# RandallBalestriero/noise-robust-vit

Hardware: AMD Instinct MI355X
Metric: images/sec (fwd+bwd+optimizer) ViT-B/16 224px bf16 (higher is better)
Workload: dtype bf16

## Files before the change

### noise_robust_vit_amd/csrc/nrv_attn.hip

```cpp
#include <type_traits>

#include "nrv_attn_common.hpp"

NRV_INTERNAL int nrv_attn_gen_supported(int B, int N, int H, int dh);
NRV_INTERNAL int nrv_attn_gen_fwd(const void* qkv, void* out, float* lse, int B, int N, int H, int dh, float scale, hipStream_t s);
NRV_INTERNAL int nrv_attn_gen_bwd(const void* qkv, const void* out, const void* dout, const float* lse, void* dqkv, float* delta_ws,
                     int B, int N, int H, int dh, float scale, hipStream_t s);
NRV_INTERNAL int nrv_attn_gen_probs(const void* qkv, const float* lse, float* probs, int B, int N, int H, int dh, float scale, hipStream_t s);

namespace {

using namespace nrv_attn;
struct AttnParams {
    const bf16_t* qkv;
    const bf16_t* out;
    const bf16_t* dout;
    bf16_t* o;
    bf16_t* dqkv;
    float* lse;
    float* delta;
    int B, N, H;
    float scale;
    long long q_rs, q_ws, q_hs, q_bs, o_rs, o_hs, o_bs;
};

void set_layout(AttnParams& p, int layout, int dh) {
    const long long T = (long long)p.B * p.N;
    if (layout & NRV_ATTN_QKV_BLOCKED) { p.q_rs = dh; p.q_ws = (long long)p.H * T * dh; p.q_hs = T * dh; p.q_bs = (long long)p.N * dh; }
    else { p.q_rs = 3ll * p.H * dh; p.q_ws = (long long)p.H * dh; p.q_hs = dh; p.q_bs = p.N * p.q_rs; }
    if (layout & NRV_ATTN_OUT_BLOCKED) { p.o_rs = dh; p.o_hs = T * dh; p.o_bs = (long long)p.N * dh; }
    else { p.o_rs = (long long)p.H * dh; p.o_hs = dh; p.o_bs = p.N * p.o_rs; }
}

template <int NT>
constexpr int atf_waves() { return NT <= 2 ? 1 : NT <= 4 ? 2 : 4; }

template <int NT>
__global__ __launch_bounds__(64 * atf_waves<NT>(), NT <= 13 ? 3 : 2) void attn_fwd_fat_kernel(const AttnParams p) {
    extern __shared__ __attribute__((aligned(16))) char smem[];
    constexpr int NP = NT * 16;
    constexpr int IMG = NP * 128;
    constexpr int NS = (NT + 1) / 2;
    constexpr int NJ = 2 * NP / 8;
    constexpr int ATF_WAVES = atf_waves<NT>();
    constexpr int JPW = NJ / ATF_WAVES;
    constexpr int MT = (NT == 13 || NT == 14) ? 1 : 2;
    const int tid = threadIdx.x, lane = tid & 63, wave = tid >> 6;
    const int N = p.N, H = p.H;
    const long long ldq = p.q_rs;
    const int b = blockIdx.x / H, h = blockIdx.x - b * H;
    const bf16_t* hb = p.qkv + (long long)b * p.q_bs + h * p.q_hs;
    const int g = lane >> 4, qc = lane & 15;
    const float sc = p.scale * LOG2E;
    const char* kimg = smem;
    const char* vimg = smem + IMG;

    const int npairs = (N + 31) >> 5;
    bf16x8_t qf[2][2];
    auto load_q = [&](int pair) {
#pragma unroll
        for (int t = 0; t < 2; ++t) {
            const int q = pair * 32 + t * 16 + qc;
            const int qr = q < N ? q : N - 1;
#pragma unroll
            for (int ks = 0; ks < 2; ++ks) qf[t][ks] = load_frag_global(hb + (long long)qr * ldq + ks * 32 + g * 8);
        }
    };
    if (wave < npairs) load_q(wave);
    {
        const __amdgpu_buffer_rsrc_t rk = make_rsrc(hb + p.q_ws, 0x7fffffffull), rv = make_rsrc(hb + 2 * p.q_ws, 0x7fffffffull);
        const int wave_u = __builtin_amdgcn_readfirstlane(wave);
#pragma unroll
        for (int i = 0; i < JPW; ++i) {
            const int j = wave_u * JPW + i;
            const bool isv = j >= NP / 8;
            const int r = 8 * (isv ? j - NP / 8 : j) + (lane >> 3);
            const int pos = lane & 7;
            const int c = isv ? ((((pos >> 1) ^ ((r >> 1) & 3)) << 1) | (pos & 1)) : (pos ^ ((r >> 1) & 7));
            const unsigned vo = (r < N) ? (unsigned)(r * ldq * 2 + c * 16) : NRV_OOB;
            if (isv) dma16_nt(rv, smem + j * 1024, vo);
            else dma16_nt(rk, smem + j * 1024, vo);
        }
    }
    __builtin_amdgcn_s_waitcnt(0x0F70);
    asm volatile("" ::: "memory");
    __syncthreads();

    const bf16x4_t zero4 = {0, 0, 0, 0};
    auto v_frag = [&](int kk, int dt) {
        const int q = (lane & 15) >> 2, pp = lane & 3;
        const int r0 = kk * 32 + 4 * g + q;
        const bf16x4_t lo = lds_read_tr16_b64(vimg + r0 * 128 + ((dt ^ ((r0 >> 1) & 3)) << 5) + pp * 8);
        if (2 * kk + 1 >= NT) return cat4(lo, zero4);
        return cat4(lo, lds_read_tr16_b64(vimg + (r0 + 16) * 128 + ((dt ^ (((r0 + 16) >> 1) & 3)) << 5) + pp * 8));
    };
    const int d_lane = (g & 1) ? 16 + 4 * (g - 1) : 4 * g;
    for (int pair = wave; pair < npairs; pair += ATF_WAVES) {
        f32x4_t st[2][NT];
        constexpr int KD = NT < 4 ? NT : 4;
        bf16x8_t kf[KD][2];
#pragma unroll
        for (int j = 0; j < KD - 1; ++j)
#pragma unroll
            for (int ks = 0; ks < 2; ++ks) kf[j][ks] = row_frag_img(kimg, j * 16, ks, lane);
#pragma unroll
        for (int kt = 0; kt < NT; ++kt) {
            if (kt + KD - 1 < NT) {
#pragma unroll
                for (int ks = 0; ks < 2; ++ks) kf[(kt + KD - 1) % KD][ks] = row_frag_img(kimg, (kt + KD - 1) * 16, ks, lane);
            }
#pragma unroll
            for (int t = 0; t < 2; ++t) {
                f32x4_t a = {0.f, 0.f, 0.f, 0.f};
#pragma unroll
                for (int ks = 0; ks < 2; ++ks) a = mfma16(kf[kt % KD][ks], qf[t][ks], a);
                st[t][kt] = a;
            }
        }
        __builtin_amdgcn_sched_barrier(0);
        const int q0 = pair * 32 + qc;
        if (pair + ATF_WAVES < npairs) load_q(pair + ATF_WAVES);
        bf16x8_t vf[2][4];
#pragma unroll
        for (int dt = 0; dt < 4; ++dt) vf[0][dt] = v_frag(0, dt);
        float m[2], l[2];
        bf16x8_t pf[2][NS];
#pragma unroll
        for (int t = 0; t < 2; ++t) {
            float mm = -INFINITY;
#pragma unroll
            for (int kt = 0; kt < NT; ++kt) {
#pragma unroll
                for (int e = 0; e < 4; ++e) {
                    if (kt >= NT - MT) mm = fmaxf(mm, (kt * 16 + 4 * g + e < N) ? st[t][kt][e] : -INFINITY);
                    else mm = fmaxf(mm, st[t][kt][e]);
                }
            }
            mm = fmaxf(mm, __shfl_xor(mm, 16, 64));
            mm = fmaxf(mm, __shfl_xor(mm, 32, 64));
            mm *= sc;
            float ll = 0.f;
#pragma unroll
            for (int kt = 0; kt < NT; ++kt) {
#pragma unroll
                for (int e = 0; e < 4; ++e) {
                    float pv = __builtin_amdgcn_exp2f(fmaf(st[t][kt][e], sc, -mm));
                    if (kt >= NT - MT) pv = (kt * 16 + 4 * g + e < N) ? pv : 0.f;
                    st[t][kt][e] = pv;
                    ll += pv;
                }
                if (kt & 1) pf[t][kt >> 1] = pack_frag(st[t][kt - 1], st[t][kt]);
                else if (kt == NT - 1) pf[t][kt >> 1] = pack_frag(st[t][kt], f32x4_t{0.f, 0.f, 0.f, 0.f});
            }
            ll += __shfl_xor(ll, 16, 64);
            ll += __shfl_xor(ll, 32, 64);
            m[t] = mm;
            l[t] = ll;
        }
        __builtin_amdgcn_sched_barrier(0);
        f32x4_t o[2][4];
#pragma unroll
        for (int t = 0; t < 2; ++t)
#pragma unroll
            for (int dt = 0; dt < 4; ++dt) o[t][dt] = f32x4_t{0.f, 0.f, 0.f, 0.f};
#pragma unroll
        for (int kk = 0; kk < NS; ++kk) {
            if (kk + 1 < NS) {
#pragma unroll
                for (int dt = 0; dt < 4; ++dt) vf[(kk + 1) & 1][dt] = v_frag(kk + 1, dt);
            }
#pragma unroll
            for (int dt = 0; dt < 4; ++dt)
#pragma unroll
                for (int t = 0; t < 2; ++t) o[t][dt] = mfma16(vf[kk & 1][dt], pf[t][kk], o[t][dt]);
        }
        __builtin_amdgcn_sched_barrier(0);
#pragma unroll
        for (int t = 0; t < 2; ++t) {
            const int q = q0 + t * 16;
            const float inv = 1.0f / l[t];
            u32x4_t ov[2];
#pragma unroll
            for (int pr = 0; pr < 2; ++pr) {
                const f32x4_t oa = o[t][2 * pr] * inv, ob = o[t][2 * pr + 1] * inv;
                const auto lo = __builtin_amdgcn_permlane16_swap(pack_bf16x2(oa[0], oa[1]), pack_bf16x2(ob[0], ob[1]), false, false);
                const auto hi = __builtin_amdgcn_permlane16_swap(pack_bf16x2(oa[2], oa[3]), pack_bf16x2(ob[2], ob[3]), false, false);
                ov[pr] = u32x4_t{lo[0], hi[0], lo[1], hi[1]};
            }
            if (q < N) {
                bf16_t* dst = p.o + (long long)b * p.o_bs + h * p.o_hs + (long long)q * p.o_rs + d_lane;
#pragma unroll
                for (int pr = 0; pr < 2; ++pr) *reinterpret_cast<u32x4_t*>(dst + 32 * pr) = ov[pr];
                if (g == 0) p.lse[((long long)b * H + h) * N + q] = (m[t] + __builtin_amdgcn_logf(l[t])) * LN2;
            }
        }
    }
}

__device__ __forceinline__ bf16x8_t row_frag_bwd(const char* img, int rb, int ks, int lane) {
    return lds_read_b128(img + vimg_off(rb + (lane & 15), ks * 4 + (lane >> 4)));
}

__device__ __forceinline__ void store_tile_bf16(bf16_t* row_ptr , const f32x4_t (&acc)[4],
                                                float mul, int g, bool ok) {
    const int d_lane = (g & 1) ? 16 + 4 * (g - 1) : 4 * g;
#pragma unroll
    for (int pr = 0; pr < 2; ++pr) {
        const f32x4_t a = acc[2 * pr] * mul, b = acc[2 * pr + 1] * mul;
        const auto lo = __builtin_amdgcn_permlane16_swap(pack_bf16x2(a[0], a[1]), pack_bf16x2(b[0], b[1]), false, false);
        const auto hi = __builtin_amdgcn_permlane16_swap(pack_bf16x2(a[2], a[3]), pack_bf16x2(b[2], b[3]), false, false);
        if (ok) *reinterpret_cast<u32x4_t*>(row_ptr + 32 * pr + d_lane) = u32x4_t{lo[0], hi[0], lo[1], hi[1]};
    }
}

template <int NT>
__device__ __forceinline__ void dma_two_images(char* smem, const bf16_t* src0, long long ld0, const bf16_t* src1, long long ld1,
                                               int N, int wave, int lane) {
    constexpr int NP = NT * 16;
    constexpr int PW = 4 * NT / atf_waves<NT>();
    const __amdgpu_buffer_rsrc_t r0 = make_rsrc(src0, 0x7fffffffull), r1 = make_rsrc(src1, 0x7fffffffull);
    const int wave_u = __builtin_amdgcn_readfirstlane(wave);
#pragma unroll
    for (int i = 0; i < PW; ++i) {
        const int j = wave_u * PW + i;
        const bool second = j >= NP / 8;
        const int r = 8 * (second ? j - NP / 8 : j) + (lane >> 3);
        const int pos = lane & 7;
        const int c = (((pos >> 1) ^ ((r >> 1) & 3)) << 1) | (pos & 1);
        const unsigned vo = (r < N) ? (unsigned)(r * (second ? ld1 : ld0) * 2 + c * 16) : NRV_OOB;
        if (second) dma16(r1, smem + j * 1024, vo);
        else dma16(r0, smem + j * 1024, vo);
    }
}

template <int NT>
__global__ __launch_bounds__(64 * atf_waves<NT>(), NT <= 13 ? 3 : 2) void attn_bwd_dq_fat_kernel(const AttnParams p) {
    extern __shared__ __attribute__((aligned(16))) char smem[];
    constexpr int ATF_WAVES = atf_waves<NT>();
    constexpr int NP = NT * 16;
    constexpr int NS = (NT + 1) / 2;
    constexpr int MT = (NT == 13 || NT == 14) ? 1 : 2;
    const char* kimg = smem;
    const char* vimg = smem + NP * 128;
    const int tid = threadIdx.x, lane = tid & 63, wave = tid >> 6;
    const int N = p.N, H = p.H;
    const int b = blockIdx.x / H, h = blockIdx.x - b * H;
    const long long ldq = p.q_rs, ldo = p.o_rs;
    const bf16_t* qbase = p.qkv + (long long)b * p.q_bs + h * p.q_hs;
    const bf16_t* obase = p.out + (long long)b * p.o_bs + h * p.o_hs;
    const bf16_t* dobase = p.dout + (long long)b * p.o_bs + h * p.o_hs;
    const int g = lane >> 4, qc = lane & 15;
    const float sc = p.scale * LOG2E;
    const int npairs = (N + 31) >> 5;

    bf16x8_t qf[2][2], dof[2][2];
    float dl[2], lse2[2];
    auto load_rows = [&](int pair) {
#pragma unroll
        for (int t = 0; t < 2; ++t) {
            const int q = pair * 32 + t * 16 + qc;
            const int qr = q < N ? q : N - 1;
            float d = 0.f;
#pragma unroll
            for (int ks = 0; ks < 2; ++ks) {
                qf[t][ks] = load_frag_global(qbase + (long long)qr * ldq + ks * 32 + g * 8);
                dof[t][ks] = load_frag_global(dobase + (long long)qr * ldo + ks * 32 + g * 8);
                const bf16x8_t of = load_frag_global(obase + (long long)qr * ldo + ks * 32 + g * 8);
#pragma unroll
                for (int e = 0; e < 8; ++e) d += bf16_to_f32((unsigned short)dof[t][ks][e]) * bf16_to_f32((unsigned short)of[e]);
            }
            d += __shfl_xor(d, 16, 64);
            d += __shfl_xor(d, 32, 64);
            dl[t] = d;
            const long long sidx = ((long long)b * H + h) * N + qr;
            lse2[t] = p.lse[sidx] * LOG2E;
            if (g == 0 && q < N) p.delta[sidx] = d;
        }
    };
    if (wave < npairs) load_rows(wave);
    dma_two_images<NT>(smem, qbase + p.q_ws, ldq, qbase + 2 * p.q_ws, ldq, N, wave, lane);
    __builtin_amdgcn_s_waitcnt(0x0F70);
    asm volatile("" ::: "memory");
    __syncthreads();

    const bf16x4_t zero4 = {0, 0, 0, 0};
    for (int pair = wave; pair < npairs; pair += ATF_WAVES) {
        f32x4_t dq[2][4];
#pragma unroll
        for (int t = 0; t < 2; ++t)
#pragma unroll
            for (int dt = 0; dt < 4; ++dt) dq[t][dt] = f32x4_t{0.f, 0.f, 0.f, 0.f};
        auto step = [&](const int kk, auto last_c) {
            constexpr bool LAST = decltype(last_c)::value;
            f32x4_t ds[2][2];
#pragma unroll
            for (int hf = 0; hf < 2; ++hf) {
                const int kt = 2 * kk + hf;
                if (!LAST || hf == 0 || (NT % 2 == 0)) {
                    bf16x8_t kr[2], vr[2];
#pragma unroll
                    for (int ks = 0; ks < 2; ++ks) {
                        kr[ks] = row_frag_bwd(kimg, kt * 16, ks, lane);
                        vr[ks] = row_frag_bwd(vimg, kt * 16, ks, lane);
                    }
#pragma unroll
                    for (int t = 0; t < 2; ++t) {
                        f32x4_t st = {0.f, 0.f, 0.f, 0.f}, dp = {0.f, 0.f, 0.f, 0.f};
#pragma unroll
                        for (int ks = 0; ks < 2; ++ks) {
                            st = mfma16(kr[ks], qf[t][ks], st);
                            dp = mfma16(vr[ks], dof[t][ks], dp);
                        }
#pragma unroll
                        for (int e = 0; e < 4; ++e) {
                            float pv = __builtin_amdgcn_exp2f(fmaf(st[e], sc, -lse2[t]));
                            if (LAST) pv = (kt * 16 + 4 * g + e < N) ? pv : 0.f;
                            ds[t][hf][e] = pv * (dp[e] - dl[t]);
                        }
                    }
                } else {
#pragma unroll
                    for (int t = 0; t < 2; ++t) ds[t][hf] = f32x4_t{0.f, 0.f, 0.f, 0.f};
                }
            }
            bf16x8_t dsf[2];
#pragma unroll
            for (int t = 0; t < 2; ++t) dsf[t] = pack_frag(ds[t][0], ds[t][1]);
#pragma unroll
            for (int dt = 0; dt < 4; ++dt) {
                const int q4 = (lane & 15) >> 2, pp = lane & 3;
                const int r0 = kk * 32 + 4 * g + q4;
                const int c = 2 * dt + (pp >> 1);
                const bf16x4_t lo = lds_read_tr16_b64(kimg + vimg_off(r0, c) + (pp & 1) * 8);
                const bf16x4_t hi = (!LAST || NT % 2 == 0) ? lds_read_tr16_b64(kimg + vimg_off(r0 + 16, c) + (pp & 1) * 8) : zero4;
                const bf16x8_t ktr = cat4(lo, hi);
#pragma unroll
                for (int t = 0; t < 2; ++t) dq[t][dt] = mfma16(ktr, dsf[t], dq[t][dt]);
            }
        };
#pragma unroll 1
        for (int kk = 0; kk < NS - 1; ++kk) step(kk, std::false_type{});
        step(NS - 1, std::true_type{});
        const int q0 = pair * 32 + qc;
        f32x4_t keep[2][4];
#pragma unroll
        for (int t = 0; t < 2; ++t)
#pragma unroll
            for (int dt = 0; dt < 4; ++dt) keep[t][dt] = dq[t][dt];
        if (pair + ATF_WAVES < npairs) load_rows(pair + ATF_WAVES);
#pragma unroll
        for (int t = 0; t < 2; ++t) {
            const int q = q0 + t * 16;
            store_tile_bf16(p.dqkv + (long long)b * p.q_bs + h * p.q_hs + (long long)(q < N ? q : 0) * ldq, keep[t], p.scale, g, q < N);
        }
    }
}

template <int NT>
__global__ __launch_bounds__(64 * atf_waves<NT>(), 2) void attn_bwd_dkv_fat_kernel(const AttnParams p) {
    extern __shared__ __attribute__((aligned(16))) char smem[];
    constexpr int ATF_WAVES = atf_waves<NT>(), ATF_THREADS = 64 * ATF_WAVES;
    constexpr int NP = NT * 16;
    constexpr int NS = (NT + 1) / 2;
    constexpr int NPS = NS * 32;
    const char* qimg = smem;
    const char* doimg = smem + NP * 128;
    float* lse2s = reinterpret_cast<float*>(smem + 2 * NP * 128);
    float* dels = lse2s + NPS;
    const int tid = threadIdx.x, lane = tid & 63, wave = tid >> 6;
    const int N = p.N, H = p.H;
    const int b = blockIdx.x / H, h = blockIdx.x - b * H;
    const long long ldq = p.q_rs, ldo = p.o_rs;
    const bf16_t* qbase = p.qkv + (long long)b * p.q_bs + h * p.q_hs;
    const bf16_t* dobase = p.dout + (long long)b * p.o_bs + h * p.o_hs;
    const int g = lane >> 4, kc = lane & 15;
    const float sc = p.scale * LOG2E;
    const int npairs = (N + 31) >> 5;

    bf16x8_t kf[2][2], vf[2][2];
    auto load_rows = [&](int pair) {
#pragma unroll
        for (int t = 0; t < 2; ++t) {
            const int key = pair * 32 + t * 16 + kc;
            const int kr = key < N ? key : N - 1;
#pragma unroll
            for (int ks = 0; ks < 2; ++ks) {
                kf[t][ks] = load_frag_global(qbase + p.q_ws + (long long)kr * ldq + ks * 32 + g * 8);
                vf[t][ks] = load_frag_global(qbase + 2 * p.q_ws + (long long)kr * ldq + ks * 32 + g * 8);
            }
        }
    };
    if (wave < npairs) load_rows(wave);
    for (int i = tid; i < NPS; i += ATF_THREADS) {
        const long long sidx = ((long long)b * H + h) * N + i;
        lse2s[i] = i < N ? p.lse[sidx] * LOG2E : INFINITY;
        dels[i] = i < N ? p.delta[sidx] : 0.f;
    }
    dma_two_images<NT>(smem, qbase, ldq, dobase, ldo, N, wave, lane);
    __builtin_amdgcn_s_waitcnt(0x0F70);
    asm volatile("" ::: "memory");
    __syncthreads();

    const bf16x4_t zero4 = {0, 0, 0, 0};
    auto tr_frag = [&](const char* img, int qq, int dt, auto last_c) {
        const int q4 = (lane & 15) >> 2, pp = lane & 3;
        const int r0 = qq * 32 + 4 * g + q4;
        const int c = 2 * dt + (pp >> 1);
        const bf16x4_t lo = lds_read_tr16_b64(img + vimg_off(r0, c) + (pp & 1) * 8);
        const bf16x4_t hi = (!decltype(last_c)::value || NT % 2 == 0) ? lds_read_tr16_b64(img + vimg_off(r0 + 16, c) + (pp & 1) * 8) : zero4;
        return cat4(lo, hi);
    };
    for (int pair = wave; pair < npairs; pair += ATF_WAVES) {
        f32x4_t dk[2][4], dv[2][4];
#pragma unroll
        for (int t = 0; t < 2; ++t)
#pragma unroll
            for (int dt = 0; dt < 4; ++dt) {
                dk[t][dt] = f32x4_t{0.f, 0.f, 0.f, 0.f};
                dv[t][dt] = dk[t][dt];
            }
        auto step = [&](const int qq, auto last_c) {
            constexpr bool LAST = decltype(last_c)::value;
            f32x4_t pt[2][2], ds[2][2];
#pragma unroll
            for (int hf = 0; hf < 2; ++hf) {
                const int qt = 2 * qq + hf;
                if (!LAST || hf == 0 || (NT % 2 == 0)) {
                    bf16x8_t qr[2], dor[2];
#pragma unroll
                    for (int ks = 0; ks < 2; ++ks) {
                        qr[ks] = row_frag_bwd(qimg, qt * 16, ks, lane);
                        dor[ks] = row_frag_bwd(doimg, qt * 16, ks, lane);
                    }
                    const f32x4_t l4 = *reinterpret_cast<const f32x4_t*>(lse2s + qt * 16 + 4 * g);
                    const f32x4_t d4 = *reinterpret_cast<const f32x4_t*>(dels + qt * 16 + 4 * g);
#pragma unroll
                    for (int t = 0; t < 2; ++t) {
                        f32x4_t st = {0.f, 0.f, 0.f, 0.f}, dp = {0.f, 0.f, 0.f, 0.f};
#pragma unroll
                        for (int ks = 0; ks < 2; ++ks) {
                            st = mfma16(qr[ks], kf[t][ks], st);
                            dp = mfma16(dor[ks], vf[t][ks], dp);
                        }
#pragma unroll
                        for (int e = 0; e < 4; ++e) {
                            const float pv = __builtin_amdgcn_exp2f(fmaf(st[e], sc, -l4[e]));
                            pt[t][hf][e] = pv;
                            ds[t][hf][e] = pv * (dp[e] - d4[e]);
                        }
                    }
                } else {
#pragma unroll
                    for (int t = 0; t < 2; ++t) {
                        pt[t][hf] = f32x4_t{0.f, 0.f, 0.f, 0.f};
                        ds[t][hf] = pt[t][hf];
                    }
                }
            }
            bf16x8_t pf[2], dsf[2];
#pragma unroll
            for (int t = 0; t < 2; ++t) {
                pf[t] = pack_frag(pt[t][0], pt[t][1]);
                dsf[t] = pack_frag(ds[t][0], ds[t][1]);
            }
#pragma unroll
            for (int dt = 0; dt < 4; ++dt) {
                const bf16x8_t dotr = tr_frag(doimg, qq, dt, last_c);
                const bf16x8_t qtr = tr_frag(qimg, qq, dt, last_c);
#pragma unroll
                for (int t = 0; t < 2; ++t) {
                    dv[t][dt] = mfma16(dotr, pf[t], dv[t][dt]);
                    dk[t][dt] = mfma16(qtr, dsf[t], dk[t][dt]);
                }
            }
        };
#pragma unroll 1
        for (int qq = 0; qq < NS - 1; ++qq) step(qq, std::false_type{});
        step(NS - 1, std::true_type{});
        const int k0 = pair * 32 + kc;
        if (pair + ATF_WAVES < npairs) load_rows(pair + ATF_WAVES);
#pragma unroll
        for (int t = 0; t < 2; ++t) {
            const int key = k0 + t * 16;
            bf16_t* row = p.dqkv + (long long)b * p.q_bs + h * p.q_hs + (long long)(key < N ? key : 0) * ldq;
            store_tile_bf16(row + p.q_ws, dk[t], p.scale, g, key < N);
            store_tile_bf16(row + 2 * p.q_ws, dv[t], 1.0f, g, key < N);
        }
    }
}

template <int NT>
int launch_fwd_fat_nt(const AttnParams& p, hipStream_t s) {
    constexpr int lds = 2 * NT * 16 * 128;
    static int attr = (int)hipFuncSetAttribute(reinterpret_cast<const void*>(attn_fwd_fat_kernel<NT>),
                                               hipFuncAttributeMaxDynamicSharedMemorySize, lds);
    if (attr != 0) return attr;
    hipLaunchKernelGGL((attn_fwd_fat_kernel<NT>), dim3(p.B * p.H), dim3(64 * atf_waves<NT>()), lds, s, p);
    NRV_CHECK_LAUNCH();
    return 0;
}

int launch_fwd_fat(const AttnParams& p, hipStream_t s) {
    const int nt = (p.N + 15) / 16;
    if (nt <= 2) return launch_fwd_fat_nt<2>(p, s);
    if (nt <= 4) return launch_fwd_fat_nt<4>(p, s);
    if (nt <= 6) return launch_fwd_fat_nt<6>(p, s);
    if (nt <= 8) return launch_fwd_fat_nt<8>(p, s);
    if (nt <= 10) return launch_fwd_fat_nt<10>(p, s);
    if (nt <= 12) return launch_fwd_fat_nt<12>(p, s);
    if (nt == 13) return launch_fwd_fat_nt<13>(p, s);
    if (nt == 14) return launch_fwd_fat_nt<14>(p, s);
    return launch_fwd_fat_nt<16>(p, s);
}

template <int NT>
int launch_bwd_fat_nt(const AttnParams& p, hipStream_t s) {
    constexpr int lds_dq = 2 * NT * 16 * 128;
    constexpr int lds_dkv = 2 * NT * 16 * 128 + 2 * ((NT + 1) / 2) * 32 * 4;
    static int a1 = (int)hipFuncSetAttribute(reinterpret_cast<const void*>(attn_bwd_dq_fat_kernel<NT>),
                                             hipFuncAttributeMaxDynamicSharedMemorySize, lds_dq);
    static int a2 = (int)hipFuncSetAttribute(reinterpret_cast<const void*>(attn_bwd_dkv_fat_kernel<NT>),
                                             hipFuncAttributeMaxDynamicSharedMemorySize, lds_dkv);
    if (a1 != 0) return a1;
    if (a2 != 0) return a2;
    hipLaunchKernelGGL((attn_bwd_dq_fat_kernel<NT>), dim3(p.B * p.H), dim3(64 * atf_waves<NT>()), lds_dq, s, p);
    NRV_CHECK_LAUNCH();
    hipLaunchKernelGGL((attn_bwd_dkv_fat_kernel<NT>), dim3(p.B * p.H), dim3(64 * atf_waves<NT>()), lds_dkv, s, p);
    NRV_CHECK_LAUNCH();
    return 0;
}

int launch_bwd_fat(const AttnParams& p, hipStream_t s) {
    const int nt = (p.N + 15) / 16;
    if (nt <= 2) return launch_bwd_fat_nt<2>(p, s);
    if (nt <= 4) return launch_bwd_fat_nt<4>(p, s);
    if (nt <= 6) return launch_bwd_fat_nt<6>(p, s);
    if (nt <= 8) return launch_bwd_fat_nt<8>(p, s);
    if (nt <= 10) return launch_bwd_fat_nt<10>(p, s);
    if (nt <= 12) return launch_bwd_fat_nt<12>(p, s);
    if (nt == 13) return launch_bwd_fat_nt<13>(p, s);
    if (nt == 14) return launch_bwd_fat_nt<14>(p, s);
    return launch_bwd_fat_nt<16>(p, s);
}

__global__ __launch_bounds__(256) void attn_probs_kernel(const AttnParams p, float* __restrict__ probs) {
    __shared__ float qs[16][DH + 1];
    const bf16_t* __restrict__ qkv = p.qkv;
    const float* __restrict__ lse = p.lse;
    const int N = p.N, H = p.H;
    const float scale = p.scale;
    const int bh = blockIdx.x, q0 = blockIdx.y * 16;
    const int b = bh / H, h = bh - b * H;
    const long long ldq = p.q_rs;
    const bf16_t* base = qkv + (long long)b * p.q_bs + h * p.q_hs;
    for (int i = threadIdx.x; i < 16 * DH; i += 256) {
        const int r = i / DH, d = i - r * DH;
        qs[r][d] = (q0 + r < N) ? bf16_to_f32(base[(long long)(q0 + r) * ldq + d]) : 0.f;
    }
    __syncthreads();
    const int qi = threadIdx.x & 15;
    const int q = q0 + qi;
    const float l = q < N ? lse[((long long)b * H + h) * N + q] : 0.f;
    for (int key = threadIdx.x >> 4; key < N; key += 16) {
        const bf16_t* kp = base + p.q_ws + (long long)key * ldq;
        float acc = 0.f;
#pragma unroll
        for (int c = 0; c < DH / 8; ++c) {
            const bf16x8_t kv = load_frag_global(kp + c * 8);
#pragma unroll
            for (int e = 0; e < 8; ++e) acc = fmaf(qs[qi][c * 8 + e], bf16_to_f32((unsigned short)kv[e]), acc);
        }
        if (q < N) probs[(((long long)b * H + h) * N + q) * N + key] = __expf(acc * scale - l);
    }
}

int shape_class(int B, int N, int H, int dh) {
    if (B <= 0 || N <= 0 || H <= 0) return 0;
    if (dh == DH && N <= 256) return (long long)B * H > 0x7fffffffll ? 0 : 1;
    return nrv_attn_gen_supported(B, N, H, dh) ? 2 : 0;
}

}

static bool layout_ok(int layout, int cls, int B, int N, int H, int dh) {
    if (layout & ~(NRV_ATTN_QKV_BLOCKED | NRV_ATTN_OUT_BLOCKED)) return false;
    if (layout != 0 && cls != 1) return false;
    return 2ll * 3 * H * (long long)B * N * dh < 0x7fffffffll;
}

extern "C" int nrv_attn_fwd(const void* qkv_bf16, void* out_bf16, float* lse,
                            int B, int N, int H, int dh, float scale, int layout, void* stream) {
    if (!qkv_bf16 || !out_bf16 || !lse) return NRV_ERR_NULL;
    const int cls = shape_class(B, N, H, dh);
    if (cls == 0 || !layout_ok(layout, cls, B, N, H, dh)) return NRV_ERR_SHAPE;
    if (!nrv_aligned16(qkv_bf16) || !nrv_aligned16(out_bf16)) return NRV_ERR_ALIGN;
    if (cls == 2) return nrv_attn_gen_fwd(qkv_bf16, out_bf16, lse, B, N, H, dh, scale, static_cast<hipStream_t>(stream));
    AttnParams p{};
    p.qkv = static_cast<const bf16_t*>(qkv_bf16);
    p.o = static_cast<bf16_t*>(out_bf16);
    p.lse = lse;
    p.B = B; p.N = N; p.H = H; p.scale = scale;
    set_layout(p, layout, dh);
    hipStream_t s = static_cast<hipStream_t>(stream);
    return launch_fwd_fat(p, s);
}

extern "C" int nrv_attn_bwd(const void* qkv_bf16, const void* out_bf16, const void* dout_bf16, const float* lse,
                            void* dqkv_bf16, float* delta_ws,
                            int B, int N, int H, int dh, float scale, int layout, void* stream) {
    if (!qkv_bf16 || !out_bf16 || !dout_bf16 || !lse || !dqkv_bf16 || !delta_ws) return NRV_ERR_NULL;
    const int cls = shape_class(B, N, H, dh);
    if (cls == 0 || !layout_ok(layout, cls, B, N, H, dh)) return NRV_ERR_SHAPE;
    if (!nrv_aligned16(qkv_bf16) || !nrv_aligned16(out_bf16) || !nrv_aligned16(dout_bf16) || !nrv_aligned16(dqkv_bf16))
        return NRV_ERR_ALIGN;
    if (cls == 2)
        return nrv_attn_gen_bwd(qkv_bf16, out_bf16, dout_bf16, lse, dqkv_bf16, delta_ws, B, N, H, dh, scale, static_cast<hipStream_t>(stream));
    AttnParams p{};
    p.qkv = static_cast<const bf16_t*>(qkv_bf16);
    p.out = static_cast<const bf16_t*>(out_bf16);
    p.dout = static_cast<const bf16_t*>(dout_bf16);
    p.dqkv = static_cast<bf16_t*>(dqkv_bf16);
    p.lse = const_cast<float*>(lse);
    p.delta = delta_ws;
    p.B = B; p.N = N; p.H = H; p.scale = scale;
    set_layout(p, layout, dh);
    hipStream_t s = static_cast<hipStream_t>(stream);
    return launch_bwd_fat(p, s);
}

extern "C" int nrv_attn_probs(const void* qkv_bf16, const float* lse, float* probs,
                              int B, int N, int H, int dh, float scale, int layout, void* stream) {
    if (!qkv_bf16 || !lse || !probs) return NRV_ERR_NULL;
    const int cls = shape_class(B, N, H, dh);
    if (cls == 0 || !layout_ok(layout, cls, B, N, H, dh)) return NRV_ERR_SHAPE;
    if (!nrv_aligned16(qkv_bf16)) return NRV_ERR_ALIGN;
    hipStream_t s = static_cast<hipStream_t>(stream);
    if (cls == 2) return nrv_attn_gen_probs(qkv_bf16, lse, probs, B, N, H, dh, scale, s);
    AttnParams p{};
    p.qkv = static_cast<const bf16_t*>(qkv_bf16);
    p.lse = const_cast<float*>(lse);
    p.B = B; p.N = N; p.H = H; p.scale = scale;
    set_layout(p, layout, dh);
    hipLaunchKernelGGL(attn_probs_kernel, dim3((unsigned)(B * H), (unsigned)((N + 15) / 16)), dim3(256), 0, s, p, probs);
    NRV_CHECK_LAUNCH();
    return 0;
}
```

Baseline: 7760.

## Fuse attention backward dQ and dK/dV kernels into one slice-pipelined kernel

Replaces the separate dQ and dK/dV backward kernels with a single kernel per (batch, head). K stays resident in LDS while Q/dO slices are double-buffered and streamed in. The softmax probabilities and dS are staged through LDS so dQ is computed per slice from the shared dS tile, instead of recomputing S and dP in a second kernel. This removes one launch and the duplicated QK^T/dO·V^T recomputation. In exchange it adds barriers per slice, needs more LDS, and drops the delta workspace write.

```diff
diff --git a/noise_robust_vit_amd/csrc/nrv_attn.hip b/noise_robust_vit_amd/csrc/nrv_attn.hip
--- a/noise_robust_vit_amd/csrc/nrv_attn.hip
+++ b/noise_robust_vit_amd/csrc/nrv_attn.hip
@@ -213,279 +213,253 @@
     }
 }
 
+template <int VMCNT>
+__device__ __forceinline__ void bwd_barrier() {
+    static_assert(VMCNT >= 0 && VMCNT < 64, "vmcnt field");
+    asm volatile("" ::: "memory");
+    __builtin_amdgcn_s_waitcnt((VMCNT & 15) | ((VMCNT >> 4) << 14) | 0x0070);
+    __builtin_amdgcn_s_barrier();
+    asm volatile("" ::: "memory");
+}
+
 template <int NT>
-__device__ __forceinline__ void dma_two_images(char* smem, const bf16_t* src0, long long ld0, const bf16_t* src1, long long ld1,
-                                               int N, int wave, int lane) {
-    constexpr int NP = NT * 16;
-    constexpr int PW = 4 * NT / atf_waves<NT>();
-    const __amdgpu_buffer_rsrc_t r0 = make_rsrc(src0, 0x7fffffffull), r1 = make_rsrc(src1, 0x7fffffffull);
-    const int wave_u = __builtin_amdgcn_readfirstlane(wave);
-#pragma unroll
-    for (int i = 0; i < PW; ++i) {
-        const int j = wave_u * PW + i;
-        const bool second = j >= NP / 8;
-        const int r = 8 * (second ? j - NP / 8 : j) + (lane >> 3);
-        const int pos = lane & 7;
-        const int c = (((pos >> 1) ^ ((r >> 1) & 3)) << 1) | (pos & 1);
-        const unsigned vo = (r < N) ? (unsigned)(r * (second ? ld1 : ld0) * 2 + c * 16) : NRV_OOB;
-        if (second) dma16(r1, smem + j * 1024, vo);
-        else dma16(r0, smem + j * 1024, vo);
-    }
-}
+struct BwdGeom {
+    static constexpr int W = atf_waves<NT>();
+    static constexpr int NP = NT * 16;
+    static constexpr int NS = (NT + 1) / 2;
+    static constexpr int TPW = (NT + W - 1) / W;
+    static constexpr int NTW = TPW * W;
+    static constexpr int DPW = 4 / W;
+    static constexpr int KIMG = NTW * 16 * 128;
+    static constexpr int SLICE = 2 * 32 * 128;
+    static constexpr int DSB = (NTW + 1) / 2 * 2 * 1024;
+    static constexpr int PB = NTW * 16 * 32;
+    static constexpr int LDS = KIMG + 2 * SLICE + DSB + PB + 2 * NTW * 16 * 4;
+};
 
 template <int NT>
-__global__ __launch_bounds__(64 * atf_waves<NT>(), NT <= 13 ? 3 : 2) void attn_bwd_dq_fat_kernel(const AttnParams p) {
+__global__ __launch_bounds__(64 * atf_waves<NT>(), 2) void attn_bwd_kernel(const AttnParams p) {
     extern __shared__ __attribute__((aligned(16))) char smem[];
-    constexpr int ATF_WAVES = atf_waves<NT>();
-    constexpr int NP = NT * 16;
-    constexpr int NS = (NT + 1) / 2;
-    constexpr int MT = (NT == 13 || NT == 14) ? 1 : 2;
-    const char* kimg = smem;
-    const char* vimg = smem + NP * 128;
-    const int tid = threadIdx.x, lane = tid & 63, wave = tid >> 6;
+    using G = BwdGeom<NT>;
+    constexpr int W = G::W, NS = G::NS, TPW = G::TPW, DPW = G::DPW;
+    char* kimg = smem;
+    char* slices = smem + G::KIMG;
+    char* dsb = slices + 2 * G::SLICE;
+    char* pb = dsb + G::DSB;
+    float* lse2s = reinterpret_cast<float*>(pb + G::PB);
+    float* dels = lse2s + G::NTW * 16;
+    const int tid = threadIdx.x, lane = tid & 63;
+    const int wave = __builtin_amdgcn_readfirstlane(tid >> 6);
     const int N = p.N, H = p.H;
     const int b = blockIdx.x / H, h = blockIdx.x - b * H;
     const long long ldq = p.q_rs, ldo = p.o_rs;
     const bf16_t* qbase = p.qkv + (long long)b * p.q_bs + h * p.q_hs;
     const bf16_t* obase = p.out + (long long)b * p.o_bs + h * p.o_hs;
     const bf16_t* dobase = p.dout + (long long)b * p.o_bs + h * p.o_hs;
-    const int g = lane >> 4, qc = lane & 15;
+    int g = lane >> 4, kc = lane & 15;
+    int q4 = kc >> 2, pp = lane & 3;
     const float sc = p.scale * LOG2E;
-    const int npairs = (N + 31) >> 5;
-
-    bf16x8_t qf[2][2], dof[2][2];
-    float dl[2], lse2[2];
-    auto load_rows = [&](int pair) {
-#pragma unroll
-        for (int t = 0; t < 2; ++t) {
-            const int q = pair * 32 + t * 16 + qc;
-            const int qr = q < N ? q : N - 1;
+    const __amdgpu_buffer_rsrc_t rq = make_rsrc(qbase, 0x7fffffffull), rdo = make_rsrc(dobase, 0x7fffffffull);
+
+    auto dma_slice = [&](int s) {
+        char* dst = slices + (s & 1) * G::SLICE;
+#pragma unroll
+        for (int i = 0; i < 8 / W; ++i) {
+            const int j = wave + i * W;
+            const bool isdo = j >= 4;
+            const int r = 8 * (j & 3) + (lane >> 3), row = s * 32 + r;
+            const int pos = lane & 7;
+            const int c = (((pos >> 1) ^ ((r >> 1) & 3)) << 1) | (pos & 1);
+            const unsigned vo = row < N ? (unsigned)(row * (isdo ? ldo : ldq) * 2 + c * 16) : NRV_OOB;
+            if (isdo) dma16(rdo, dst + j * 1024, vo);
+            else dma16(rq, dst + j * 1024, vo);
+        }
+    };
+    {
+        const __amdgpu_buffer_rsrc_t rk = make_rsrc(qbase + p.q_ws, 0x7fffffffull);
+        for (int j = wave; j < G::NTW * 2; j += W) {
+            const int r = 8 * j + (lane >> 3), pos = lane & 7;
+            const int c = (((pos >> 1) ^ ((r >> 1) & 3)) << 1) | (pos & 1);
+            dma16(rk, kimg + j * 1024, r < N ? (unsigned)(r * ldq * 2 + c * 16) : NRV_OOB);
+        }
+        dma_slice(0);
+    }
+    bf16x8_t vf[TPW][2];
+#pragma unroll
+    for (int tw = 0; tw < TPW; ++tw) {
+        const int kr = min((wave + tw * W) * 16 + kc, N - 1);
+#pragma unroll
+        for (int ks = 0; ks < 2; ++ks) vf[tw][ks] = load_frag_global(qbase + 2 * p.q_ws + (long long)kr * ldq + ks * 32 + g * 8);
+    }
+    {
+        bf16x8_t dof[TPW][2], of[TPW][2];
+        float lq[TPW];
+#pragma unroll
+        for (int tw = 0; tw < TPW; ++tw) {
+            const int rr = min((wave + tw * W) * 16 + kc, N - 1);
+#pragma unroll
+            for (int ks = 0; ks < 2; ++ks) {
+                dof[tw][ks] = load_frag_global(dobase + (long long)rr * ldo + ks * 32 + g * 8);
+                of[tw][ks] = load_frag_global(obase + (long long)rr * ldo + ks * 32 + g * 8);
+            }
+            lq[tw] = p.lse[((long long)b * H + h) * N + rr];
+        }
+#pragma unroll
+        for (int tw = 0; tw < TPW; ++tw) {
+            const int row = (wave + tw * W) * 16 + kc;
             float d = 0.f;
 #pragma unroll
-            for (int ks = 0; ks < 2; ++ks) {
-                qf[t][ks] = load_frag_global(qbase + (long long)qr * ldq + ks * 32 + g * 8);
-                dof[t][ks] = load_frag_global(dobase + (long long)qr * ldo + ks * 32 + g * 8);
-                const bf16x8_t of = load_frag_global(obase + (long long)qr * ldo + ks * 32 + g * 8);
-#pragma unroll
-                for (int e = 0; e < 8; ++e) d += bf16_to_f32((unsigned short)dof[t][ks][e]) * bf16_to_f32((unsigned short)of[e]);
-            }
+            for (int ks = 0; ks < 2; ++ks)
+#pragma unroll
+                for (int e = 0; e < 8; ++e) d += bf16_to_f32((unsigned short)dof[tw][ks][e]) * bf16_to_f32((unsigned short)of[tw][ks][e]);
             d += __shfl_xor(d, 16, 64);
             d += __shfl_xor(d, 32, 64);
-            dl[t] = d;
-            const long long sidx = ((long long)b * H + h) * N + qr;
-            lse2[t] = p.lse[sidx] * LOG2E;
-            if (g == 0 && q < N) p.delta[sidx] = d;
-        }
-    };
-    if (wave < npairs) load_rows(wave);
-    dma_two_images<NT>(smem, qbase + p.q_ws, ldq, qbase + 2 * p.q_ws, ldq, N, wave, lane);
-    __builtin_amdgcn_s_waitcnt(0x0F70);
-    asm volatile("" ::: "memory");
-    __syncthreads();
+            if (g == 0) {
+                lse2s[row] = row < N ? lq[tw] * LOG2E : INFINITY;
+                dels[row] = row < N ? d : 0.f;
+            }
+        }
+    }
+    bwd_barrier<0>();
+
+    bool kval[TPW];
+#pragma unroll
+    for (int tw = 0; tw < TPW; ++tw) kval[tw] = (wave + tw * W) * 16 + kc < N;
+    f32x4_t dk[TPW][4], dv[TPW][4];
+#pragma unroll
+    for (int tw = 0; tw < TPW; ++tw)
+#pragma unroll
+        for (int dt = 0; dt < 4; ++dt) {
+            dk[tw][dt] = f32x4_t{0.f, 0.f, 0.f, 0.f};
+            dv[tw][dt] = dk[tw][dt];
+        }
 
     const bf16x4_t zero4 = {0, 0, 0, 0};
-    for (int pair = wave; pair < npairs; pair += ATF_WAVES) {
-        f32x4_t dq[2][4];
-#pragma unroll
-        for (int t = 0; t < 2; ++t)
-#pragma unroll
-            for (int dt = 0; dt < 4; ++dt) dq[t][dt] = f32x4_t{0.f, 0.f, 0.f, 0.f};
-        auto step = [&](const int kk, auto last_c) {
-            constexpr bool LAST = decltype(last_c)::value;
-            f32x4_t ds[2][2];
-#pragma unroll
-            for (int hf = 0; hf < 2; ++hf) {
-                const int kt = 2 * kk + hf;
-                if (!LAST || hf == 0 || (NT % 2 == 0)) {
-                    bf16x8_t kr[2], vr[2];
-#pragma unroll
-                    for (int ks = 0; ks < 2; ++ks) {
-                        kr[ks] = row_frag_bwd(kimg, kt * 16, ks, lane);
-                        vr[ks] = row_frag_bwd(vimg, kt * 16, ks, lane);
-                    }
-#pragma unroll
-                    for (int t = 0; t < 2; ++t) {
-                        f32x4_t st = {0.f, 0.f, 0.f, 0.f}, dp = {0.f, 0.f, 0.f, 0.f};
-#pragma unroll
-                        for (int ks = 0; ks < 2; ++ks) {
-                            st = mfma16(kr[ks], qf[t][ks], st);
-                            dp = mfma16(vr[ks], dof[t][ks], dp);
-                        }
-#pragma unroll
-                        for (int e = 0; e < 4; ++e) {
-                            float pv = __builtin_amdgcn_exp2f(fmaf(st[e], sc, -lse2[t]));
-                            if (LAST) pv = (kt * 16 + 4 * g + e < N) ? pv : 0.f;
-                            ds[t][hf][e] = pv * (dp[e] - dl[t]);
-                        }
-                    }
-                } else {
-#pragma unroll
-                    for (int t = 0; t < 2; ++t) ds[t][hf] = f32x4_t{0.f, 0.f, 0.f, 0.f};
-                }
-            }
-            bf16x8_t dsf[2];
-#pragma unroll
-            for (int t = 0; t < 2; ++t) dsf[t] = pack_frag(ds[t][0], ds[t][1]);
-#pragma unroll
-            for (int dt = 0; dt < 4; ++dt) {
-                const int q4 = (lane & 15) >> 2, pp = lane & 3;
-                const int r0 = kk * 32 + 4 * g + q4;
-                const int c = 2 * dt + (pp >> 1);
-                const bf16x4_t lo = lds_read_tr16_b64(kimg + vimg_off(r0, c) + (pp & 1) * 8);
-                const bf16x4_t hi = (!LAST || NT % 2 == 0) ? lds_read_tr16_b64(kimg + vimg_off(r0 + 16, c) + (pp & 1) * 8) : zero4;
-                const bf16x8_t ktr = cat4(lo, hi);
-#pragma unroll
-                for (int t = 0; t < 2; ++t) dq[t][dt] = mfma16(ktr, dsf[t], dq[t][dt]);
-            }
-        };
-#pragma unroll 1
-        for (int kk = 0; kk < NS - 1; ++kk) step(kk, std::false_type{});
-        step(NS - 1, std::true_type{});
-        const int q0 = pair * 32 + qc;
-        f32x4_t keep[2][4];
-#pragma unroll
-        for (int t = 0; t < 2; ++t)
-#pragma unroll
-            for (int dt = 0; dt < 4; ++dt) keep[t][dt] = dq[t][dt];
-        if (pair + ATF_WAVES < npairs) load_rows(pair + ATF_WAVES);
-#pragma unroll
-        for (int t = 0; t < 2; ++t) {
-            const int q = q0 + t * 16;
-            store_tile_bf16(p.dqkv + (long long)b * p.q_bs + h * p.q_hs + (long long)(q < N ? q : 0) * ldq, keep[t], p.scale, g, q < N);
-        }
-    }
-}
-
-template <int NT>
-__global__ __launch_bounds__(64 * atf_waves<NT>(), 2) void attn_bwd_dkv_fat_kernel(const AttnParams p) {
-    extern __shared__ __attribute__((aligned(16))) char smem[];
-    constexpr int ATF_WAVES = atf_waves<NT>(), ATF_THREADS = 64 * ATF_WAVES;
-    constexpr int NP = NT * 16;
-    constexpr int NS = (NT + 1) / 2;
-    constexpr int NPS = NS * 32;
-    const char* qimg = smem;
-    const char* doimg = smem + NP * 128;
-    float* lse2s = reinterpret_cast<float*>(smem + 2 * NP * 128);
-    float* dels = lse2s + NPS;
-    const int tid = threadIdx.x, lane = tid & 63, wave = tid >> 6;
-    const int N = p.N, H = p.H;
-    const int b = blockIdx.x / H, h = blockIdx.x - b * H;
-    const long long ldq = p.q_rs, ldo = p.o_rs;
-    const bf16_t* qbase = p.qkv + (long long)b * p.q_bs + h * p.q_hs;
-    const bf16_t* dobase = p.dout + (long long)b * p.o_bs + h * p.o_hs;
-    const int g = lane >> 4, kc = lane & 15;
-    const float sc = p.scale * LOG2E;
-    const int npairs = (N + 31) >> 5;
-
-    bf16x8_t kf[2][2], vf[2][2];
-    auto load_rows = [&](int pair) {
-#pragma unroll
-        for (int t = 0; t < 2; ++t) {
-            const int key = pair * 32 + t * 16 + kc;
-            const int kr = key < N ? key : N - 1;
-#pragma unroll
-            for (int ks = 0; ks < 2; ++ks) {
-                kf[t][ks] = load_frag_global(qbase + p.q_ws + (long long)kr * ldq + ks * 32 + g * 8);
-                vf[t][ks] = load_frag_global(qbase + 2 * p.q_ws + (long long)kr * ldq + ks * 32 + g * 8);
-            }
-        }
-    };
-    if (wave < npairs) load_rows(wave);
-    for (int i = tid; i < NPS; i += ATF_THREADS) {
-        const long long sidx = ((long long)b * H + h) * N + i;
-        lse2s[i] = i < N ? p.lse[sidx] * LOG2E : INFINITY;
-        dels[i] = i < N ? p.delta[sidx] : 0.f;
-    }
-    dma_two_images<NT>(smem, qbase, ldq, dobase, ldo, N, wave, lane);
-    __builtin_amdgcn_s_waitcnt(0x0F70);
-    asm volatile("" ::: "memory");
-    __syncthreads();
-
-    const bf16x4_t zero4 = {0, 0, 0, 0};
-    auto tr_frag = [&](const char* img, int qq, int dt, auto last_c) {
-        const int q4 = (lane & 15) >> 2, pp = lane & 3;
-        const int r0 = qq * 32 + 4 * g + q4;
+    auto tr_frag = [&](const char* img, int rb, int dt, auto hi_c) {
+        const int r0 = rb + 4 * g + q4;
         const int c = 2 * dt + (pp >> 1);
         const bf16x4_t lo = lds_read_tr16_b64(img + vimg_off(r0, c) + (pp & 1) * 8);
-        const bf16x4_t hi = (!decltype(last_c)::value || NT % 2 == 0) ? lds_read_tr16_b64(img + vimg_off(r0 + 16, c) + (pp & 1) * 8) : zero4;
+        const bf16x4_t hi = decltype(hi_c)::value ? lds_read_tr16_b64(img + vimg_off(r0 + 16, c) + (pp & 1) * 8) : zero4;
         return cat4(lo, hi);
     };
-    for (int pair = wave; pair < npairs; pair += ATF_WAVES) {
-        f32x4_t dk[2][4], dv[2][4];
-#pragma unroll
-        for (int t = 0; t < 2; ++t)
-#pragma unroll
-            for (int dt = 0; dt < 4; ++dt) {
-                dk[t][dt] = f32x4_t{0.f, 0.f, 0.f, 0.f};
-                dv[t][dt] = dk[t][dt];
-            }
-        auto step = [&](const int qq, auto last_c) {
-            constexpr bool LAST = decltype(last_c)::value;
-            f32x4_t pt[2][2], ds[2][2];
-#pragma unroll
-            for (int hf = 0; hf < 2; ++hf) {
-                const int qt = 2 * qq + hf;
-                if (!LAST || hf == 0 || (NT % 2 == 0)) {
-                    bf16x8_t qr[2], dor[2];
-#pragma unroll
-                    for (int ks = 0; ks < 2; ++ks) {
-                        qr[ks] = row_frag_bwd(qimg, qt * 16, ks, lane);
-                        dor[ks] = row_frag_bwd(doimg, qt * 16, ks, lane);
-                    }
-                    const f32x4_t l4 = *reinterpret_cast<const f32x4_t*>(lse2s + qt * 16 + 4 * g);
-                    const f32x4_t d4 = *reinterpret_cast<const f32x4_t*>(dels + qt * 16 + 4 * g);
-#pragma unroll
-                    for (int t = 0; t < 2; ++t) {
+    auto ds_slot = [&](int tile, int hf) { return dsb + ((tile >> 1) * 2 + hf) * 1024 + ((tile & 1) * 16 + kc) * 32 + g * 8; };
+    auto p_slot = [&](int tile) { return pb + (tile * 16 + kc) * 32 + g * 8; };
+    auto step = [&](const int s, auto last_c) {
+        constexpr bool LAST = decltype(last_c)::value;
+        constexpr int NH = (LAST && NT % 2) ? 1 : 2;
+        const char* qs = slices + (s & 1) * G::SLICE;
+        const char* dos = qs + G::SLICE / 2;
+        if (!LAST) dma_slice(s + 1);
+        u32x2_t pk[TPW];
+#pragma unroll
+        for (int hf = 0; hf < 2; ++hf) {
+            if (hf < NH) {
+                bf16x8_t qr[2], dor[2];
+#pragma unroll
+                for (int ks = 0; ks < 2; ++ks) {
+                    qr[ks] = row_frag_bwd(qs, hf * 16, ks, lane);
+                    dor[ks] = row_frag_bwd(dos, hf * 16, ks, lane);
+                }
+                const f32x4_t l4 = *reinterpret_cast<const f32x4_t*>(lse2s + s * 32 + hf * 16 + 4 * g);
+                const f32x4_t d4 = *reinterpret_cast<const f32x4_t*>(dels + s * 32 + hf * 16 + 4 * g);
+#pragma unroll
+                for (int tw = 0; tw < TPW; ++tw) {
+                    {
+                        const int tile = wave + tw * W;
                         f32x4_t st = {0.f, 0.f, 0.f, 0.f}, dp = {0.f, 0.f, 0.f, 0.f};
 #pragma unroll
                         for (int ks = 0; ks < 2; ++ks) {
-                            st = mfma16(qr[ks], kf[t][ks], st);
-                            dp = mfma16(dor[ks], vf[t][ks], dp);
+                            st = mfma16(qr[ks], row_frag_bwd(kimg, tile * 16, ks, lane), st);
+                            dp = mfma16(dor[ks], vf[tw][ks], dp);
                         }
+                        f32x4_t pt, ds;
 #pragma unroll
                         for (int e = 0; e < 4; ++e) {
-                            const float pv = __builtin_amdgcn_exp2f(fmaf(st[e], sc, -l4[e]));
-                            pt[t][hf][e] = pv;
-                            ds[t][hf][e] = pv * (dp[e] - d4[e]);
+                            float pv = __builtin_amdgcn_exp2f(fmaf(st[e], sc, -l4[e]));
+                            pv = kval[tw] ? pv : 0.f;
+                            pt[e] = pv;
+                            ds[e] = pv * (dp[e] - d4[e]);
                         }
-                    }
-                } else {
-#pragma unroll
-                    for (int t = 0; t < 2; ++t) {
-                        pt[t][hf] = f32x4_t{0.f, 0.f, 0.f, 0.f};
-                        ds[t][hf] = pt[t][hf];
+                        const u32x2_t pv2 = {pack_bf16x2(pt[0], pt[1]), pack_bf16x2(pt[2], pt[3])};
+                        if (hf == 0) *reinterpret_cast<u32x2_t*>(p_slot(tile)) = pv2;
+                        else pk[tw] = pv2;
+                        store_bf16x4(reinterpret_cast<bf16_t*>(ds_slot(tile, hf)), ds);
                     }
                 }
-            }
-            bf16x8_t pf[2], dsf[2];
-#pragma unroll
-            for (int t = 0; t < 2; ++t) {
-                pf[t] = pack_frag(pt[t][0], pt[t][1]);
-                dsf[t] = pack_frag(ds[t][0], ds[t][1]);
-            }
-#pragma unroll
-            for (int dt = 0; dt < 4; ++dt) {
-                const bf16x8_t dotr = tr_frag(doimg, qq, dt, last_c);
-                const bf16x8_t qtr = tr_frag(qimg, qq, dt, last_c);
-#pragma unroll
-                for (int t = 0; t < 2; ++t) {
-                    dv[t][dt] = mfma16(dotr, pf[t], dv[t][dt]);
-                    dk[t][dt] = mfma16(qtr, dsf[t], dk[t][dt]);
+            } else {
+#pragma unroll
+                for (int tw = 0; tw < TPW; ++tw) pk[tw] = u32x2_t{0u, 0u};
+            }
+        }
+        using HasHi = std::integral_constant<bool, NH == 2>;
+#pragma unroll
+        for (int dt = 0; dt < 4; ++dt) {
+            const bf16x8_t dotr = tr_frag(dos, 0, dt, HasHi{});
+#pragma unroll
+            for (int tw = 0; tw < TPW; ++tw) {
+                {
+                    const u32x2_t p0 = *reinterpret_cast<const u32x2_t*>(p_slot(wave + tw * W));
+                    const bf16x8_t pf = __builtin_bit_cast(bf16x8_t, u32x4_t{p0[0], p0[1], pk[tw][0], pk[tw][1]});
+                    dv[tw][dt] = mfma16(dotr, pf, dv[tw][dt]);
                 }
             }
-        };
+        }
+        bf16x8_t dsf[TPW];
+#pragma unroll
+        for (int tw = 0; tw < TPW; ++tw) {
+            const int tile = wave + tw * W;
+            const u32x2_t d0 = *reinterpret_cast<const u32x2_t*>(ds_slot(tile, 0));
+            const u32x2_t d1 = NH == 2 ? *reinterpret_cast<const u32x2_t*>(ds_slot(tile, 1)) : u32x2_t{0u, 0u};
+            dsf[tw] = __builtin_bit_cast(bf16x8_t, u32x4_t{d0[0], d0[1], d1[0], d1[1]});
+        }
+#pragma unroll
+        for (int dt = 0; dt < 4; ++dt) {
+            const bf16x8_t qtr = tr_frag(qs, 0, dt, HasHi{});
+#pragma unroll
+            for (int tw = 0; tw < TPW; ++tw)
+                dk[tw][dt] = mfma16(qtr, dsf[tw], dk[tw][dt]);
+        }
+        bwd_barrier<63>();
+#pragma unroll
+        for (int j = 0; j < DPW; ++j) {
+            const int dt = wave + j * W;
+            f32x4_t acc[2] = {{0.f, 0.f, 0.f, 0.f}, {0.f, 0.f, 0.f, 0.f}};
+#pragma unroll
+            for (int kk = 0; kk < NS; ++kk) {
+                const bool full = !(kk == NS - 1 && NT % 2);
+                bf16x8_t ktr;
+                if (full) ktr = tr_frag(kimg, kk * 32, dt, std::true_type{});
+                else ktr = tr_frag(kimg, kk * 32, dt, std::false_type{});
+#pragma unroll
+                for (int hf = 0; hf < NH; ++hf) {
+                    const char* pa = dsb + (kk * 2 + hf) * 1024 + (4 * g + q4) * 32 + pp * 8;
+                    const bf16x8_t dst = cat4(lds_read_tr16_b64(pa), full ? lds_read_tr16_b64(pa + 16 * 32) : zero4);
+                    acc[hf] = mfma16(ktr, dst, acc[hf]);
+                }
+            }
+#pragma unroll
+            for (int hf = 0; hf < NH; ++hf) {
+                const int q = s * 32 + hf * 16 + kc;
+                bf16_t* dst = p.dqkv + (long long)b * p.q_bs + h * p.q_hs + (long long)q * ldq + 16 * dt + 4 * g;
+                if (!LAST || q < N) store_bf16x4(dst, acc[hf] * p.scale);
+            }
+        }
+        if (!LAST) bwd_barrier<2 * DPW>();
+    };
 #pragma unroll 1
-        for (int qq = 0; qq < NS - 1; ++qq) step(qq, std::false_type{});
-        step(NS - 1, std::true_type{});
-        const int k0 = pair * 32 + kc;
-        if (pair + ATF_WAVES < npairs) load_rows(pair + ATF_WAVES);
-#pragma unroll
-        for (int t = 0; t < 2; ++t) {
-            const int key = k0 + t * 16;
-            bf16_t* row = p.dqkv + (long long)b * p.q_bs + h * p.q_hs + (long long)(key < N ? key : 0) * ldq;
-            store_tile_bf16(row + p.q_ws, dk[t], p.scale, g, key < N);
-            store_tile_bf16(row + 2 * p.q_ws, dv[t], 1.0f, g, key < N);
-        }
+    for (int s = 0; s < NS - 1; ++s) step(s, std::false_type{});
+    {
+        const int ln = (int)__builtin_amdgcn_mbcnt_hi(~0u, __builtin_amdgcn_mbcnt_lo(~0u, 0u));
+        g = ln >> 4; kc = ln & 15; q4 = kc >> 2; pp = ln & 3;
+    }
+    step(NS - 1, std::true_type{});
+
+#pragma unroll
+    for (int tw = 0; tw < TPW; ++tw) {
+        const int key = (wave + tw * W) * 16 + kc;
+        bf16_t* row = p.dqkv + (long long)b * p.q_bs + h * p.q_hs + (long long)(key < N ? key : 0) * ldq;
+        store_tile_bf16(row + p.q_ws, dk[tw], p.scale, g, key < N);
+        store_tile_bf16(row + 2 * p.q_ws, dv[tw], 1.0f, g, key < N);
     }
 }
 
@@ -514,33 +488,28 @@
 }
 
 template <int NT>
-int launch_bwd_fat_nt(const AttnParams& p, hipStream_t s) {
-    constexpr int lds_dq = 2 * NT * 16 * 128;
-    constexpr int lds_dkv = 2 * NT * 16 * 128 + 2 * ((NT + 1) / 2) * 32 * 4;
-    static int a1 = (int)hipFuncSetAttribute(reinterpret_cast<const void*>(attn_bwd_dq_fat_kernel<NT>),
-                                             hipFuncAttributeMaxDynamicSharedMemorySize, lds_dq);
-    static int a2 = (int)hipFuncSetAttribute(reinterpret_cast<const void*>(attn_bwd_dkv_fat_kernel<NT>),
-                                             hipFuncAttributeMaxDynamicSharedMemorySize, lds_dkv);
-    if (a1 != 0) return a1;
-    if (a2 != 0) return a2;
-    hipLaunchKernelGGL((attn_bwd_dq_fat_kernel<NT>), dim3(p.B * p.H), dim3(64 * atf_waves<NT>()), lds_dq, s, p);
-    NRV_CHECK_LAUNCH();
-    hipLaunchKernelGGL((attn_bwd_dkv_fat_kernel<NT>), dim3(p.B * p.H), dim3(64 * atf_waves<NT>()), lds_dkv, s, p);
+int launch_bwd_nt(const AttnParams& p, hipStream_t s) {
+    constexpr int lds = BwdGeom<NT>::LDS;
+    static_assert(lds <= 80 * 1024, "two workgroups per CU");
+    static int attr = (int)hipFuncSetAttribute(reinterpret_cast<const void*>(attn_bwd_kernel<NT>),
+                                               hipFuncAttributeMaxDynamicSharedMemorySize, lds);
+    if (attr != 0) return attr;
+    hipLaunchKernelGGL((attn_bwd_kernel<NT>), dim3(p.B * p.H), dim3(64 * atf_waves<NT>()), lds, s, p);
     NRV_CHECK_LAUNCH();
     return 0;
 }
 
-int launch_bwd_fat(const AttnParams& p, hipStream_t s) {
+int launch_bwd(const AttnParams& p, hipStream_t s) {
     const int nt = (p.N + 15) / 16;
-    if (nt <= 2) return launch_bwd_fat_nt<2>(p, s);
-    if (nt <= 4) return launch_bwd_fat_nt<4>(p, s);
-    if (nt <= 6) return launch_bwd_fat_nt<6>(p, s);
-    if (nt <= 8) return launch_bwd_fat_nt<8>(p, s);
-    if (nt <= 10) return launch_bwd_fat_nt<10>(p, s);
-    if (nt <= 12) return launch_bwd_fat_nt<12>(p, s);
-    if (nt == 13) return launch_bwd_fat_nt<13>(p, s);
-    if (nt == 14) return launch_bwd_fat_nt<14>(p, s);
-    return launch_bwd_fat_nt<16>(p, s);
+    if (nt <= 2) return launch_bwd_nt<2>(p, s);
+    if (nt <= 4) return launch_bwd_nt<4>(p, s);
+    if (nt <= 6) return launch_bwd_nt<6>(p, s);
+    if (nt <= 8) return launch_bwd_nt<8>(p, s);
+    if (nt <= 10) return launch_bwd_nt<10>(p, s);
+    if (nt <= 12) return launch_bwd_nt<12>(p, s);
+    if (nt == 13) return launch_bwd_nt<13>(p, s);
+    if (nt == 14) return launch_bwd_nt<14>(p, s);
+    return launch_bwd_nt<16>(p, s);
 }
 
 __global__ __launch_bounds__(256) void attn_probs_kernel(const AttnParams p, float* __restrict__ probs) {
@@ -625,7 +594,7 @@
     p.B = B; p.N = N; p.H = H; p.scale = scale;
     set_layout(p, layout, dh);
     hipStream_t s = static_cast<hipStream_t>(stream);
-    return launch_bwd_fat(p, s);
+    return launch_bwd(p, s);
 }
 
 extern "C" int nrv_attn_probs(const void* qkv_bf16, const float* lse, float* probs,
```

Result: no change. 7837 (median of 6 runs) (+1.0%).
